# aaletov/open-pcc-metric

Hardware: AMD Instinct MI355X
Metric: Mpoints/s for symmetric D1+D2 PSNR, N_ref=N_deg=1M (higher is better)
Workload: dtype f64

## Files before the change

include/pccm.h:

```cpp
#ifndef PCCM_H
#define PCCM_H

#include <stdint.h>

#ifdef __cplusplus
extern "C" {
#endif

#define PCCM_VERSION 100

#define PCCM_OK 0
#define PCCM_E_ARG (-1)
#define PCCM_E_NODEV (-2)
#define PCCM_E_HIP (-3)
#define PCCM_E_OOM (-4)
#define PCCM_E_STATE (-5)
#define PCCM_E_RANGE (-6)

#define PCCM_F32 0
#define PCCM_F64 1

#define PCCM_DIR_LEFT 0
#define PCCM_DIR_RIGHT 1
#define PCCM_DIR_SELF 2
// ... 56 lines not shown
int pccm_nn_want_idx(pccm_ctx *ctx, int on);

int pccm_nn_fetch(pccm_ctx *ctx, int dir, int32_t *idx, double *d2);

int pccm_error_vectors(pccm_ctx *ctx, int dir, double *out);

int pccm_tie_exposure(pccm_ctx *ctx, int dir, int normal_mode, double out[8]);

int pccm_point_metric(pccm_ctx *ctx, int dir, int metric, int normal_mode, double *out);

int64_t pccm_xvec_len(int64_t n_iter);
int pccm_reduce_prefetch(pccm_ctx *ctx, int dir, int metric, int normal_mode);
int pccm_reduce_prefetch_many(pccm_ctx *ctx, int n, const int *dirs, const int *metrics, const int *normal_modes);
int pccm_reduce(pccm_ctx *ctx, int dir, int metric, int normal_mode, double *xvec, double *minmax);
int pccm_finish_sum(const double *xvec, int64_t n_iter, double *sum);
int pccm_reduce_total(pccm_ctx *ctx, int dir, int metric, int normal_mode, double out[3]);
int pccm_reduce_total_many(pccm_ctx *ctx, int n, const int *dirs, const int *metrics, const int *normal_modes, double *out);

int64_t pccm_cvec_len(int64_t n_iter);
int pccm_reduce_chunks_many(pccm_ctx *ctx, int n, const int *dirs, const int *metrics, const int *normal_modes, double *cvecs,
                            double *minmax);
int pccm_finish_chunks(const double *cvec, int64_t n_iter, double *sum);

int pccm_set_colors(pccm_ctx *ctx, int which, const void *rgb, int64_t n, int dtype, int on_device);

int pccm_set_colors_u8(pccm_ctx *ctx, int which, const unsigned char *rgb, int64_t n);

int pccm_color_reduce(pccm_ctx *ctx, int dir, int scheme, double scale, const int32_t *rows, int64_t nrows,
                      double sum_out[3], double max_out[3]);

int pccm_color_rows(pccm_ctx *ctx, int dir, int scheme, double scale, int what, const int32_t *rows, int64_t nrows,
                    double *out);

int pccm_obb_frames(pccm_ctx *ctx, const double *verts, int64_t nv, const double *tri, int64_t nt, double ext_out[3], double *vol_out);

int pccm_extreme_rows(pccm_ctx *ctx, int which, const float *dirs, int ndirs, int32_t *rows_out);
int pccm_rows_outside(pccm_ctx *ctx, int which, const double *planes, int nplanes, double margin, int32_t *rows_out, int64_t *count);

int pccm_seq_colsum(pccm_ctx *ctx, const double *cols, int64_t n, double out[3]);

int pccm_lzf_decompress(const unsigned char *in, int64_t in_len, unsigned char *out, int64_t out_cap, int64_t *out_len);

int pccm_color_transform(const double *rgb, int64_t n, int scheme, double *out);

int pccm_drop_caches(pccm_ctx *ctx);

// ... 19 lines not shown
```

open_pcc_metric_amd/_native.py:

```python
from __future__ import annotations

import ctypes
import os
import sys
import threading
from typing import Optional, Tuple

import numpy as np

_HERE = os.path.dirname(os.path.abspath(__file__))
LIB_PATH = os.environ.get("PCCM_LIB") or os.path.join(_HERE, "csrc", "libpccm.so")

OK, E_ARG, E_NODEV, E_HIP, E_OOM, E_STATE, E_RANGE = 0, -1, -2, -3, -4, -5, -6
F32, F64 = 0, 1
DIR_LEFT, DIR_RIGHT, DIR_SELF = 0, 1, 2
ENGINES = {"auto": 0, "brute": 1, "grid": 2}
NORMAL_MODES = {"row": 0, "neighbour": 1}
METRIC_D1, METRIC_D2, METRIC_PROJ = 0, 1, 2
KERNEL_CLASSES = {"ingest": 0, "scan": 1, "refine": 2, "fallback": 3, "point": 4, "reduce": 5,
                  "grid_build": 6, "grid_query": 7, "grid_finish": 8}

SYMBOLS = (
    "pccm_version", "pccm_last_error", "pccm_device_count", "pccm_ctx_create", "pccm_ctx_destroy", "pccm_ctx_reset",
    "pccm_set_cloud", "pccm_set_normals", "pccm_set_normals_deferred", "pccm_flush_uploads", "pccm_set_io_staged", "pccm_estimate_normals", "pccm_get_normals", "pccm_set_shard", "pccm_set_shard_dir", "pccm_shard_range", "pccm_nn", "pccm_nn_pair", "pccm_nn_fuse", "pccm_nn_want_idx", "pccm_nn_fetch",
    "pccm_error_vectors", "pccm_point_metric", "pccm_tie_exposure", "pccm_xvec_len", "pccm_reduce_prefetch", "pccm_reduce_prefetch_many", "pccm_reduce", "pccm_finish_sum",
    "pccm_reduce_total", "pccm_reduce_total_many", "pccm_cvec_len", "pccm_reduce_chunks_many", "pccm_finish_chunks",
    "pccm_set_colors", "pccm_set_colors_u8", "pccm_color_reduce", "pccm_color_rows", "pccm_seq_colsum", "pccm_obb_frames", "pccm_extreme_rows", "pccm_rows_outside",
    "pccm_color_transform", "pccm_lzf_decompress", "pccm_drop_caches", "pccm_graph_begin", "pccm_graph_end", "pccm_graph_launch", "pccm_graph_destroy",
    "pccm_sync",
    "pccm_profile_enable", "pccm_profile_reset", "pccm_profile_get", "pccm_nn_stats",
)

COLOR_SCHEMES = {"rgb": 0, "ycc": 1, "yuv": 2}
COLOR_OWN, COLOR_NEIGHBOUR, COLOR_DIFF, COLOR_SQUARE = 0, 1, 2, 3

_lib = None


class NativeLibraryMissing(ImportError):
    pass


class PccmStateError(RuntimeError):
    """PCCM_E_STATE: a call came in the wrong order or hit a stale object (a hipGraph captured before buffers
    changed, a reduction before its search).  The context is intact; callers may recover (CloudPair re-captures)."""


class PccmDeviceError(RuntimeError):
    """PCCM_E_HIP / PCCM_E_NODEV: the HIP runtime reported a failure.  Never retried, never swallowed."""
# ... 6 lines not shown
    if not os.path.exists(LIB_PATH):
        raise NativeLibraryMissing(
            f"{LIB_PATH} is not built: open_pcc_metric_amd has no CPU fallback. "
            "Run `make -C open_pcc_metric_amd/csrc` (needs hipcc, --offload-arch=gfx950).")
    if "torch" in sys.modules or os.environ.get("PCCM_NO_TORCH") != "1":
        try:
            import torch
        except ImportError:
            pass
    lib = ctypes.CDLL(LIB_PATH)
    vp, i32, i64 = ctypes.c_void_p, ctypes.c_int, ctypes.c_int64
    dp = ctypes.POINTER(ctypes.c_double)
    lib.pccm_version.restype = i32
    lib.pccm_last_error.restype = ctypes.c_char_p
    lib.pccm_device_count.argtypes = [ctypes.POINTER(i32)]
    lib.pccm_ctx_create.argtypes = [i32, vp, ctypes.POINTER(vp)]
    lib.pccm_ctx_destroy.argtypes = [vp]
    lib.pccm_ctx_reset.argtypes = [vp]
    lib.pccm_set_cloud.argtypes = [vp, i32, vp, i64, i32, i32]
    lib.pccm_set_normals.argtypes = [vp, i32, vp, i64, i32, i32]
    lib.pccm_set_normals_deferred.argtypes = [vp, i32, vp, i64, i32]
    lib.pccm_flush_uploads.argtypes = [vp]
    lib.pccm_set_io_staged.argtypes = [vp, i32]
    lib.pccm_set_shard.argtypes = [vp, i32, i32]
    lib.pccm_set_shard_dir.argtypes = [vp, i32, i32, i32]
    lib.pccm_estimate_normals.argtypes = [vp, i32, i32]
    lib.pccm_get_normals.argtypes = [vp, i32, vp]
    lib.pccm_shard_range.argtypes = [vp, i32, ctypes.POINTER(i64), ctypes.POINTER(i64)]
    lib.pccm_nn.argtypes = [vp, i32, i32]
    lib.pccm_nn_pair.argtypes = [vp, i32]
    lib.pccm_nn_fuse.argtypes = [vp, i32, i32]
    lib.pccm_nn_want_idx.argtypes = [vp, i32]
    lib.pccm_nn_fetch.argtypes = [vp, i32, vp, vp]
    lib.pccm_error_vectors.argtypes = [vp, i32, vp]
    lib.pccm_point_metric.argtypes = [vp, i32, i32, i32, vp]
    lib.pccm_tie_exposure.argtypes = [vp, i32, i32, dp]
    lib.pccm_xvec_len.argtypes = [i64]
    lib.pccm_xvec_len.restype = i64
    lib.pccm_reduce.argtypes = [vp, i32, i32, i32, vp, vp]
    lib.pccm_reduce_prefetch.argtypes = [vp, i32, i32, i32]
    ip = ctypes.POINTER(i32)
    lib.pccm_reduce_prefetch_many.argtypes = [vp, i32, ip, ip, ip]
    lib.pccm_finish_sum.argtypes = [vp, i64, dp]
    lib.pccm_reduce_total.argtypes = [vp, i32, i32, i32, dp]
    lib.pccm_reduce_total_many.argtypes = [vp, i32, ip, ip, ip, dp]
    lib.pccm_cvec_len.argtypes = [i64]
# ... 200 lines not shown
        self._n = [0, 0]

    def set_cloud(self, which: int, points) -> None:
        ptr, n, dt, dev, keep = _as_rows(points, "points")
        _check(self._lib.pccm_set_cloud(self._ctx, int(which), ptr, n, dt, dev))
        self._n[which] = n

    def set_normals(self, which: int, normals) -> None:
        ptr, n, dt, dev, keep = _as_rows(normals, "normals")
        self.__dict__.setdefault("_deferred", {}).pop(int(which), None)
        _check(self._lib.pccm_set_normals(self._ctx, int(which), ptr, n, dt, dev))

    def set_normals_deferred(self, which: int, normals) -> None:
        ptr, n, dt, dev, keep = _as_rows(normals, "normals")
        if dev:
            _check(self._lib.pccm_set_normals(self._ctx, int(which), ptr, n, dt, dev))
            return
        _check(self._lib.pccm_set_normals_deferred(self._ctx, int(which), ptr, n, dt))
        self.__dict__.setdefault("_deferred", {})[int(which)] = keep

    def set_io_staged(self, on: bool) -> None:
        _check(self._lib.pccm_set_io_staged(self._ctx, 1 if on else 0))

    def flush_uploads(self) -> None:
        try:
            _check(self._lib.pccm_flush_uploads(self._ctx))
        finally:
            self.__dict__.get("_deferred", {}).clear()

    def set_colors(self, which: int, colors) -> None:
        ptr, n, dt, dev, keep = _as_rows(colors, "colors")
        _check(self._lib.pccm_set_colors(self._ctx, int(which), ptr, n, dt, dev))

    def set_colors_u8(self, which: int, colors_u8) -> None:
        c = np.ascontiguousarray(colors_u8, dtype=np.uint8)
        if c.ndim != 2 or c.shape[1] != 3:
            raise ValueError("colors_u8 must have shape (N, 3)")
        _check(self._lib.pccm_set_colors_u8(self._ctx, int(which), c.ctypes.data_as(ctypes.c_void_p), c.shape[0]))

    @staticmethod
    def _rows_arg(rows):
        if rows is None:
            return None, 0, None
        keep = np.ascontiguousarray(rows, dtype=np.int32)
        return keep.ctypes.data_as(ctypes.c_void_p), keep.shape[0], keep

# ... 200 lines not shown
```

open_pcc_metric_amd/csrc/pccm_api.hip:

```cpp
#include <math.h>
#include <stdarg.h>
#include <stdio.h>
#include <string.h>

#include <new>
#include <thread>

#include "pccm_internal.h"

namespace pccm {

static thread_local char g_err[512] = "";

int fail(int code, const char *fmt, ...)
{
    va_list ap;
    va_start(ap, fmt);
    vsnprintf(g_err, sizeof(g_err), fmt, ap);
    va_end(ap);
    return code;
}

int ensure(pccm_ctx *ctx, DevBuf &b, size_t bytes)
{
    if (bytes <= b.bytes && b.p) return PCCM_OK;
    if (ctx->capturing) {
        ctx->capture_failed = true;
// ... 356 lines not shown
    if (!out) return fail(PCCM_E_ARG, "null pointer");
    *out = nullptr;
    int c = 0;
    if (hipGetDeviceCount(&c) != hipSuccess || c <= 0) {
        (void)hipGetLastError();
        return fail(PCCM_E_NODEV, "no HIP device is visible: libpccm has no CPU path");
    }
    if (device < 0 || device >= c) return fail(PCCM_E_ARG, "device %d out of range (0..%d)", device, c - 1);
    PCCM_HIP(hipSetDevice(device));
    pccm_ctx *ctx = new (std::nothrow) pccm_ctx();
    if (!ctx) return fail(PCCM_E_OOM, "host allocation failed");
    ctx->device = device;
    if (hip_stream) {
        ctx->stream = (hipStream_t)hip_stream;
    } else {
        hipError_t e = hipStreamCreateWithFlags(&ctx->stream, hipStreamNonBlocking);
        if (e != hipSuccess) {
            delete ctx;
            return fail(PCCM_E_HIP, "hipStreamCreate: %s", hipGetErrorString(e));
        }
        ctx->own_stream = true;
    }
    int rc = ensure(ctx, ctx->counters, 16 * sizeof(uint32_t));
    if (!rc && hipHostMalloc((void **)&ctx->host_err, 64, hipHostMallocDefault) != hipSuccess) {
        ctx->host_err = nullptr;
        rc = fail(PCCM_E_OOM, "hipHostMalloc of the device error word failed");
    }
    if (!rc) *ctx->host_err = 0u;
    if (!rc && hipEventCreateWithFlags(&ctx->batch_ev, hipEventDisableTiming) != hipSuccess) rc = fail(PCCM_E_HIP, "hipEventCreate failed");
    if (!rc) rc = ensure(ctx, ctx->stats, 32 * sizeof(unsigned long long));
    if (!rc && hipMemsetAsync(ctx->counters.p, 0, 16 * sizeof(uint32_t), ctx->stream) != hipSuccess)
        rc = fail(PCCM_E_HIP, "hipMemsetAsync failed");
    if (rc) {
        pccm_ctx_destroy(ctx);
        return rc;
    }
    for (int d = 0; d < 3; ++d) ctx->nn[d].nflag_dev = (uint32_t *)ctx->counters.p + 2 * d;
    *out = ctx;
    return PCCM_OK;
}

int pccm_ctx_destroy(pccm_ctx *ctx)
{
    if (!ctx) return PCCM_OK;
    (void)hipSetDevice(ctx->device);
    if (ctx->stream) (void)hipStreamSynchronize(ctx->stream);
    for (auto &s : ctx->spans) {
        (void)hipEventDestroy(s.a);
        (void)hipEventDestroy(s.b);
    }
    for (auto e : ctx->event_pool) (void)hipEventDestroy(e);
    if (ctx->batch_ev) (void)hipEventDestroy(ctx->batch_ev);
    ctx->batch_ev = nullptr;
    if (ctx->host_err) (void)hipHostFree(ctx->host_err);
    ctx->host_err = nullptr;
    for (int k = 0; k < 2; ++k) free_cloud(ctx->cloud[k]);
    for (int d = 0; d < 3; ++d) free_nn(ctx->nn[d]);
    DevBuf *bufs[] = {&ctx->part_b1, &ctx->part_g, &ctx->part_b2, &ctx->val, &ctx->stats, &ctx->staging, &ctx->staging2,
                      &ctx->counters, &ctx->color_cols, &ctx->color_idx, &ctx->colsum_scratch, &ctx->rescan_part, &ctx->tail_sync};
    for (DevBuf *b : bufs) free_buf(*b);
    for (auto &g : ctx->graphs) graph_free(g);
    for (auto &s : ctx->slots) {
        free_buf(s.val);
        if (s.host) (void)hipHostFree(s.host);
        if (s.ev) (void)hipEventDestroy(s.ev);
        s.ev = s.wait_ev = nullptr;
    }
    grid_release(ctx);
    if (ctx->copy_stream) (void)hipStreamDestroy(ctx->copy_stream);
    for (auto &pbuf : ctx->pin)
        if (pbuf) (void)hipHostFree(pbuf);
    for (auto &pe : ctx->pin_ev)
        if (pe) (void)hipEventDestroy(pe);
    if (ctx->own_stream && ctx->stream) (void)hipStreamDestroy(ctx->stream);
    delete ctx;
    return PCCM_OK;
}

// ... 85 lines not shown
    if (!nrm || n <= 0) return fail(PCCM_E_ARG, "empty normals");
    if (dtype != PCCM_F32 && dtype != PCCM_F64) return fail(PCCM_E_ARG, "dtype must be PCCM_F32 or PCCM_F64");
    Cloud &c = ctx->cloud[which];
    PCCM_HIP(hipStreamSynchronize(ctx->stream));
    for (int d = 0; d < 3; ++d) ctx->nn_gen[d]++;
    ctx->epoch++;
    c.nrm_exact32 = false;
    int rc = grow((void **)&c.nrm64, c.cap_nrm, (size_t)n * 3 * sizeof(double));
    if (rc) return rc;
    if ((rc = grow((void **)&c.nrm32, c.cap_nrm32, (size_t)n * sizeof(float4)))) return rc;
    c.n_nrm = n;
    c.nrm_host = nrm;
    c.nrm_host_dtype = dtype;
    c.nrm_deferred = true;
    return PCCM_OK;
}

int pccm_set_io_staged(pccm_ctx *ctx, int on)
{
    CHECK_CTX(ctx);
    NOT_CAPTURING(ctx);
    PCCM_HIP(hipStreamSynchronize(ctx->stream));
    ctx->io_staged = on != 0;
    return PCCM_OK;
}

int pccm_flush_uploads(pccm_ctx *ctx)
{
    CHECK_CTX(ctx);
    NOT_CAPTURING(ctx);
    for (int k = 0; k < 2; ++k) {
        int rc = normals_ready(ctx, ctx->cloud[k]);
        if (rc) return rc;
    }
    return PCCM_OK;
}

int pccm_set_colors(pccm_ctx *ctx, int which, const void *rgb, int64_t n, int dtype, int on_device)
{
    CHECK_CTX(ctx);
    NOT_CAPTURING(ctx);
    if (which != 0 && which != 1) return fail(PCCM_E_ARG, "cloud index must be 0 or 1");
    if (!rgb || n <= 0) return fail(PCCM_E_ARG, "empty colours");
    if (dtype != PCCM_F32 && dtype != PCCM_F64) return fail(PCCM_E_ARG, "dtype must be PCCM_F32 or PCCM_F64");
    Cloud &c = ctx->cloud[which];
    if (c.n == 0) return fail(PCCM_E_STATE, "set cloud %d before its colours", which);
// ... 584 lines not shown
    return tie_exposure(ctx, dir, *it, *se, *res, normal_mode, out);
}

int pccm_point_metric(pccm_ctx *ctx, int dir, int metric, int normal_mode, double *out)
{
    CHECK_CTX(ctx);
    NOT_CAPTURING(ctx);
    if (!out) return fail(PCCM_E_ARG, "null pointer");
    const double *dev;
    int64_t ns;
    const Cloud *it;
    NNResult *res;
    int rc = metric_on_device(ctx, dir, metric, normal_mode, &dev, &ns, &it, &res);
    if (rc) return rc;
    if (ns > 0) { int rcd = d2h(ctx, out, dev, (size_t)ns * sizeof(double)); if (rcd) return rcd; }
    PCCM_HIP(hipStreamSynchronize(ctx->stream));
    return PCCM_OK;
}

int64_t pccm_xvec_len(int64_t n_iter)
{
    if (n_iter <= 0) return 0;
    return (n_iter / kChunk) * (kChunk / kLeaf) + (n_iter % kChunk);
}

static int slot_prepare(pccm_ctx *ctx, ReduceSlot &s, int dir, int metric, int normal_mode, bool want_units, PointJobs &pj,
                        UnitJobs &uj)
{
    const Cloud *it, *se;
    NNResult *res;
    int rc = need_nn(ctx, dir, &it, &se, &res);
    if (rc) return rc;
    const int64_t ns = res->end - res->begin;
    const double *dev = nullptr;
    int stride = 1, square = 0, defer = 0;
    if (metric == PCCM_METRIC_D1) {
        if (res->rec_valid) {
            dev = (const double *)res->rec.p;
            stride = res->rec_stride;
            if (res->rec_layout == 1) defer = 3;
        } else {
            if ((rc = ensure_plain(ctx, *res, false))) return rc;
            dev = res->d2;
        }
    } else {
        if (metric != PCCM_METRIC_D2 && metric != PCCM_METRIC_PROJ) return fail(PCCM_E_ARG, "bad metric %d", metric);
// ... 17 lines not shown
                pj.off[pj.njobs + 1] = pj.off[pj.njobs] + ns;
                pj.njobs++;
            }
        }
    }
    s.dir = dir; s.metric = metric; s.mode = normal_mode;
    s.gen = ctx->nn_gen[dir];
    s.n_iter = it->n; s.begin = res->begin; s.end = res->end;
    s.nunits = ns > 0 ? (ns + kLeaf - 1) / kLeaf : 0;
    s.nblocks = (s.nunits + 31) / 32;
    s.has_units = want_units;
    const int64_t nfull = it->n / kChunk, full_rows = nfull * kChunk;
    s.t0 = res->begin > full_rows ? res->begin : full_rows;
    s.tail_n = s.t0 < res->end ? res->end - s.t0 : 0;
    const size_t need = (size_t)(3 * s.nunits + 3 * s.nblocks + s.tail_n + 1) * sizeof(double);
    if (ctx->capturing && (need > s.host_cap || !s.ev)) {
        ctx->capture_failed = true;
        return fail(PCCM_E_STATE, "a reduction slot must be allocated during graph capture: run the sequence once first");
    }
    if (need > s.host_cap) {
        ctx->epoch++;
        if (s.host) (void)hipHostFree(s.host);
        s.host = nullptr; s.host_cap = 0;
        PCCM_HIP(hipHostMalloc((void **)&s.host, need, hipHostMallocDefault));
        s.host_cap = need;
    }
    if (!s.ev) PCCM_HIP(hipEventCreateWithFlags(&s.ev, hipEventDisableTiming));
    if (s.nunits > 0) {
        UnitCol col;
        col.off = (stride >= 2 && metric != PCCM_METRIC_D1) ? 1 : 0;
        col.square = square;
        col.out_units = want_units ? s.host : nullptr;
        col.out_blocks = s.host + 3 * s.nunits;
        col.out_tail = s.host + 3 * s.nunits + 3 * s.nblocks;
        const double *base = stride >= 2 ? (const double *)res->rec.p : dev;
        UnitJob *host_job = nullptr;
        static const bool merge = [] {
            const char *e = PCCM_DIAG_ENV("PCCM_REDUCE_MERGE");
            return !(e && e[0] == '0');
        }();
        if (stride >= 2 && merge)
            for (int k = 0; k < uj.njobs; ++k)
                if (uj.j[k].stride >= 2 && uj.j[k].val == base && uj.j[k].ncols == 1 &&
                    (uj.j[k].defer == defer || uj.j[k].defer == 3 || defer == 3))
                    host_job = &uj.j[k];
        if (host_job) {
            host_job->c[1] = col;
// ... 57 lines not shown
static int prefetch_many(pccm_ctx *ctx, int n, const int *dirs, const int *metrics, const int *normal_modes, bool want_units)
{
    if (n < 0 || n > 8 || (n > 0 && (!dirs || !metrics || !normal_modes))) return fail(PCCM_E_ARG, "1..8 requests expected");
    PointJobs pj;
    UnitJobs uj;
    pj.njobs = 0; pj.off[0] = 0;
    uj.njobs = 0; uj.uoff[0] = 0; uj.toff[0] = 0;
    ReduceSlot *fresh[8];
    int nfresh = 0;
    for (int k = 0; k < n; ++k) {
        if (dirs[k] < 0 || dirs[k] > 2) return fail(PCCM_E_ARG, "bad direction %d", dirs[k]);
        if (metrics[k] == PCCM_METRIC_D1 || dirs[k] == PCCM_DIR_SELF) continue;
        NNResult &res = ctx->nn[dirs[k]];
        if (!res.valid || !res.rec_valid || ((res.fused_mode == normal_modes[k] || res.rec_stride == 4 || res.rec_layout == 1) && !res.no_rows)) continue;
        if (slot_find(ctx, dirs[k], metrics[k], normal_modes[k], want_units)) continue;
        int rc = ensure_plain(ctx, res, true);
        if (rc) return rc;
    }
    for (int k = 0; k < n; ++k) {
        if (dirs[k] < 0 || dirs[k] > 2) return fail(PCCM_E_ARG, "bad direction %d", dirs[k]);
        if (slot_find(ctx, dirs[k], metrics[k], normal_modes[k], want_units)) continue;
        ReduceSlot *s = slot_free(ctx, fresh, nfresh);
        if (!s) return fail(PCCM_E_STATE, "no free reduction slot: more than 8 live columns in one batch");
        if (s->pending && !ctx->capturing && s->wait_ev) PCCM_HIP(hipEventSynchronize(s->wait_ev));
        s->pending = false;
        int rc = slot_prepare(ctx, *s, dirs[k], metrics[k], normal_modes[k], want_units, pj, uj);
        if (rc) return rc;
        s->pending = true;
        fresh[nfresh++] = s;
    }
    if (nfresh == 0) return PCCM_OK;
    int rc;
    if ((rc = launch_point_jobs(ctx, pj))) return rc;
    if ((rc = launch_unit_jobs(ctx, uj))) return rc;
    for (int k = 0; k < nfresh; ++k) {
        ReduceSlot &s = *fresh[k];
        if (ctx->capturing) {
            GraphOp op;
            op.kind = 2;
            op.dir = s.dir;
            op.slot = (int)(&s - ctx->slots);
            op.snap = s;
            ctx->cap_ops.push_back(op);
        } else {
            s.wait_ev = ctx->batch_ev;
        }
    }
    if (!ctx->capturing) PCCM_HIP(hipEventRecord(ctx->batch_ev, ctx->stream));
    return PCCM_OK;
}

int pccm_reduce_prefetch(pccm_ctx *ctx, int dir, int metric, int normal_mode)
{
    return pccm_reduce_prefetch_many(ctx, 1, &dir, &metric, &normal_mode);
}

int pccm_reduce(pccm_ctx *ctx, int dir, int metric, int normal_mode, double *xvec, double *minmax)
{
    CHECK_CTX(ctx);
    NOT_CAPTURING(ctx);
    if (!xvec || !minmax) return fail(PCCM_E_ARG, "null pointer");
    if (dir < 0 || dir > 2) return fail(PCCM_E_ARG, "bad direction %d", dir);
    ReduceSlot *s = slot_find(ctx, dir, metric, normal_mode, true);
    if (!s) {
        int rc = prefetch_many(ctx, 1, &dir, &metric, &normal_mode, true);
        if (rc) return rc;
        s = slot_find(ctx, dir, metric, normal_mode, true);
        if (!s) return fail(PCCM_E_STATE, "reduction slot lost");
    }
    if (s->wait_ev) PCCM_HIP(hipEventSynchronize(s->wait_ev));
    { int rce = check_device_errors(ctx); if (rce) return rce; }
    s->pending = false;
    const int64_t n = s->n_iter;
    const int64_t xlen = pccm_xvec_len(n);
    memset(xvec, 0, (size_t)xlen * sizeof(double));
    minmax[0] = INFINITY;
    minmax[1] = -INFINITY;
    const int64_t nunits = s->nunits;
    const int64_t nfull = n / kChunk, full_rows = nfull * kChunk;
    const double *usum = s->host, *umin = usum + nunits, *umax = usum + 2 * nunits;
    for (int64_t u = 0; u < nunits; ++u) {
        const int64_t row = s->begin + u * kLeaf;
        if (row < full_rows) xvec[row / kLeaf] = usum[u];
        if (umin[u] < minmax[0]) minmax[0] = umin[u];
        if (umax[u] > minmax[1]) minmax[1] = umax[u];
    }
    if (s->tail_n > 0)
        memcpy(xvec + nfull * (kChunk / kLeaf) + (s->t0 - full_rows), s->host + 3 * nunits + 3 * s->nblocks,
               (size_t)s->tail_n * sizeof(double));
    return PCCM_OK;
}

static double leaf_tree(const double *l, int cnt)
// ... 12 lines not shown
    for (int64_t c = 0; c < nfull; ++c) {
        double cs = leaf_tree(xvec + c * lpc, lpc);
        s = first ? cs : s + cs;
        first = false;
    }
    if (tail) {
        double ts = np_pairwise_sum(xvec + nfull * lpc, tail);
        s = first ? ts : s + ts;
    }
    *sum = s;
    return PCCM_OK;
}

static int total_from_slot(pccm_ctx *ctx, int dir, int metric, int normal_mode, double out[3])
{
    if (dir < 0 || dir > 2) return fail(PCCM_E_ARG, "bad direction %d", dir);
    ReduceSlot *s = slot_find(ctx, dir, metric, normal_mode);
    if (!s) {
        int rc = pccm_reduce_prefetch(ctx, dir, metric, normal_mode);
        if (rc) return rc;
        s = slot_find(ctx, dir, metric, normal_mode);
        if (!s) return fail(PCCM_E_STATE, "reduction slot lost");
    }
    if (s->wait_ev) PCCM_HIP(hipEventSynchronize(s->wait_ev));
    { int rce = check_device_errors(ctx); if (rce) return rce; }
    s->pending = false;
    const int64_t n = s->n_iter, nunits = s->nunits, nblocks = s->nblocks;
    const int64_t nfull = n / kChunk;
    const double *bsum = s->host + 3 * nunits, *bmin = bsum + nblocks, *bmax = bsum + 2 * nblocks;
    double total = 0.0;
    bool first = true;
    for (int64_t c = 0; c < nfull; ++c) {
        const double cs = bsum[2 * c] + bsum[2 * c + 1];
        total = first ? cs : total + cs;
        first = false;
    }
    if (s->tail_n > 0) {
        const double ts = np_pairwise_sum(s->host + 3 * nunits + 3 * nblocks, s->tail_n);
        total = first ? ts : total + ts;
    }
    double mn = INFINITY, mx = -INFINITY;
    for (int64_t b = 0; b < nblocks; ++b) {
        mn = bmin[b] < mn ? bmin[b] : mn;
        mx = bmax[b] > mx ? bmax[b] : mx;
    }
    out[0] = total;
    out[1] = mn;
    out[2] = mx;
    return PCCM_OK;
}

int64_t pccm_cvec_len(int64_t n_iter)
{
    if (n_iter <= 0) return 0;
    return n_iter / kChunk + n_iter % kChunk;
}

static int chunks_from_slot(pccm_ctx *ctx, int dir, int metric, int normal_mode, double *cvec, double minmax[2])
{
    if (dir < 0 || dir > 2) return fail(PCCM_E_ARG, "bad direction %d", dir);
    ReduceSlot *s = slot_find(ctx, dir, metric, normal_mode);
    if (!s) {
        int rc = prefetch_many(ctx, 1, &dir, &metric, &normal_mode, false);
        if (rc) return rc;
        s = slot_find(ctx, dir, metric, normal_mode);
        if (!s) return fail(PCCM_E_STATE, "reduction slot lost");
    }
    if (s->wait_ev) PCCM_HIP(hipEventSynchronize(s->wait_ev));
    { int rce = check_device_errors(ctx); if (rce) return rce; }
    s->pending = false;
    const int64_t n = s->n_iter, nunits = s->nunits, nblocks = s->nblocks;
    const int64_t nfull = n / kChunk, full_rows = nfull * kChunk;
    memset(cvec, 0, (size_t)pccm_cvec_len(n) * sizeof(double));
    minmax[0] = INFINITY;
    minmax[1] = -INFINITY;
    if (s->end <= s->begin) return PCCM_OK;
    if (s->begin % kChunk != 0 || (s->end % kChunk != 0 && s->end != n))
        return fail(PCCM_E_STATE, "rows [%lld, %lld) do not start and end on 8192-row chunks: use pccm_reduce", (long long)s->begin,
                    (long long)s->end);
    const double *bsum = s->host + 3 * nunits, *bmin = bsum + nblocks, *bmax = bsum + 2 * nblocks;
    const int64_t c0 = s->begin / kChunk;
    const int64_t owned = ((s->end < full_rows ? s->end : full_rows) - s->begin) / kChunk;
    for (int64_t c = 0; c < owned; ++c) cvec[c0 + c] = bsum[2 * c] + bsum[2 * c + 1];
    if (s->tail_n > 0)
        memcpy(cvec + nfull + (s->t0 - full_rows), s->host + 3 * nunits + 3 * nblocks, (size_t)s->tail_n * sizeof(double));
    for (int64_t b = 0; b < nblocks; ++b) {
        minmax[0] = bmin[b] < minmax[0] ? bmin[b] : minmax[0];
        minmax[1] = bmax[b] > minmax[1] ? bmax[b] : minmax[1];
    }
    return PCCM_OK;
}
// ... 125 lines not shown
    if (g.graph) (void)hipGraphDestroy(g.graph);
    g.exec = nullptr;
    g.graph = nullptr;
    g.valid = false;
    g.ops.clear();
}

static int graph_replay(pccm_ctx *ctx, GraphRec &g)
{

    for (auto &op : g.ops) {
        if (op.kind == 1) {
            ctx->nn_gen[op.dir]++;
            ctx->nn[op.dir].valid = true;
            ctx->nn[op.dir].rec_valid = op.rec_valid;
            ctx->nn[op.dir].plain_valid = op.plain_valid;
            ctx->nn[op.dir].fused_mode = op.fused_mode;
            ctx->nn[op.dir].rec_stride = op.rec_stride;
            ctx->nn[op.dir].rec_layout = op.rec_layout;
            ctx->nn[op.dir].no_rows = op.no_rows;
            ctx->nn[op.dir].plain_d2_valid = op.plain_valid;
        } else if (op.kind == 2) {
            ReduceSlot &s = ctx->slots[op.slot];
            if (s.pending && s.gen == ctx->nn_gen[s.dir] && s.wait_ev) PCCM_HIP(hipEventSynchronize(s.wait_ev));
            s.dir = op.snap.dir; s.metric = op.snap.metric; s.mode = op.snap.mode;
            s.n_iter = op.snap.n_iter; s.begin = op.snap.begin; s.end = op.snap.end;
            s.nunits = op.snap.nunits; s.nblocks = op.snap.nblocks; s.has_units = op.snap.has_units;
            s.t0 = op.snap.t0; s.tail_n = op.snap.tail_n;
            s.gen = ctx->nn_gen[s.dir];
            s.pending = true;
            s.wait_ev = ctx->batch_ev;
        }
    }
    PCCM_HIP(hipGraphLaunch(g.exec, ctx->stream));
    PCCM_HIP(hipEventRecord(ctx->batch_ev, ctx->stream));
    return PCCM_OK;
}

int pccm_graph_begin(pccm_ctx *ctx)
{
    CHECK_CTX(ctx);
    if (ctx->capturing) return fail(PCCM_E_STATE, "already capturing");
    PCCM_HIP(hipStreamSynchronize(ctx->stream));
    for (auto &s : ctx->slots) s.pending = false;
    ctx->cap_ops.clear();
    ctx->capture_failed = false;
    PCCM_HIP(hipStreamBeginCapture(ctx->stream, hipStreamCaptureModeThreadLocal));
    ctx->capturing = true;
    return PCCM_OK;
}

int pccm_graph_end(pccm_ctx *ctx, int *graph_id)
{
    CHECK_CTX(ctx);
    if (!graph_id) return fail(PCCM_E_ARG, "null pointer");
    if (!ctx->capturing) return fail(PCCM_E_STATE, "pccm_graph_begin was not called");
    ctx->capturing = false;
    GraphRec g;
    hipError_t e = hipStreamEndCapture(ctx->stream, &g.graph);
    if (e != hipSuccess || ctx->capture_failed || !g.graph) {
        (void)hipGetLastError();
        if (g.graph) (void)hipGraphDestroy(g.graph);
        for (int d = 0; d < 3; ++d) { ctx->nn[d].valid = false; ctx->nn_gen[d]++; }
        for (auto &s : ctx->slots) s.pending = false;
        grid_invalidate(ctx);
        return fail(PCCM_E_STATE, "graph capture failed (%s); the context is usable, results were invalidated",
                    e != hipSuccess ? hipGetErrorString(e) : "a captured call reported an error");
    }
    e = hipGraphInstantiate(&g.exec, g.graph, nullptr, nullptr, 0);
    if (e != hipSuccess) {
        (void)hipGraphDestroy(g.graph);
        for (int d = 0; d < 3; ++d) { ctx->nn[d].valid = false; ctx->nn_gen[d]++; }
        for (auto &s : ctx->slots) s.pending = false;
        grid_invalidate(ctx);
        return fail(PCCM_E_HIP, "hipGraphInstantiate: %s", hipGetErrorString(e));
    }
    g.ops = ctx->cap_ops;
    for (auto &op : g.ops)
        if (op.kind == 1) {
            op.rec_valid = ctx->nn[op.dir].rec_valid;
            op.plain_valid = ctx->nn[op.dir].plain_valid;
            op.fused_mode = ctx->nn[op.dir].fused_mode;
            op.rec_stride = ctx->nn[op.dir].rec_stride;
            op.rec_layout = ctx->nn[op.dir].rec_layout;
            op.no_rows = ctx->nn[op.dir].no_rows;
        }
    g.epoch = ctx->epoch;
    g.valid = true;
    PCCM_HIP(hipGraphLaunch(g.exec, ctx->stream));
    for (auto &op : g.ops)
        if (op.kind == 2) ctx->slots[op.slot].wait_ev = ctx->batch_ev;
    PCCM_HIP(hipEventRecord(ctx->batch_ev, ctx->stream));
    int id = -1;
    for (size_t k = 0; k < ctx->graphs.size(); ++k)
        if (!ctx->graphs[k].valid && !ctx->graphs[k].exec) { id = (int)k; break; }
    if (id < 0) { ctx->graphs.emplace_back(); id = (int)ctx->graphs.size() - 1; }
    ctx->graphs[id] = g;
    *graph_id = id;
    return PCCM_OK;
}

int pccm_graph_launch(pccm_ctx *ctx, int graph_id)
{
    CHECK_CTX(ctx);
    NOT_CAPTURING(ctx);
    if (graph_id < 0 || graph_id >= (int)ctx->graphs.size() || !ctx->graphs[graph_id].valid)
        return fail(PCCM_E_ARG, "unknown graph %d", graph_id);
    GraphRec &g = ctx->graphs[graph_id];
    if (g.epoch != ctx->epoch) {
        graph_free(g);
        return fail(PCCM_E_STATE, "graph %d is stale: inputs, shard or buffers changed since it was captured", graph_id);
    }
    return graph_replay(ctx, g);
}
// ... 111 lines not shown
```

open_pcc_metric_amd/csrc/pccm_internal.h:

```cpp
#pragma once
#include <hip/hip_runtime.h>
#include <stdint.h>
#include <mutex>
#include <string>
#include <vector>

#include "pccm.h"

#ifdef PCCM_DIAG
#define PCCM_DIAG_ENV(name) getenv(name)
#else
#define PCCM_DIAG_ENV(name) (static_cast<const char *>(nullptr))
#endif

namespace pccm {

constexpr int kScanThreads = 256;
constexpr int kScanTile = 1024;
constexpr int kTileVec = kScanTile / 4 * 3;
constexpr int kGranule = 64;
constexpr float kBig32 = 3.0e38f;
constexpr float kPadCoord = 1.0e18f;
constexpr double kMaxAbsCoord = 1.0e15;

// ... 105 lines not shown
    bool lattice = false;
    DevBuf occ;
    DevBuf recs;
    bool vox = false;
    DevBuf vbricks;
    DevBuf vlist;
    DevBuf vcount;
    bool vox_rows = false;
    uint64_t vox_rows_pair = 0;
    DevBuf vminrow;
};

struct ReduceSlot {
    bool pending = false;
    int dir = 0, metric = 0, mode = 0;
    uint64_t gen = 0;
    int64_t n_iter = 0, begin = 0, end = 0, nunits = 0, nblocks = 0, t0 = 0, tail_n = 0;
    bool has_units = false;
    DevBuf val;
    double *host = nullptr;
    size_t host_cap = 0;
    hipEvent_t ev = nullptr;
    hipEvent_t wait_ev = nullptr;
};

struct ProfSpan {
    hipEvent_t a, b;
    int cls;
};

struct GraphOp {
    int kind = 0;
    int dir = 0, slot = -1;
    bool rec_valid = false, plain_valid = false;
    int fused_mode = -1, rec_stride = 4, rec_layout = 0;
    bool no_rows = false;
    ReduceSlot snap;
};

struct GraphRec {
    hipGraph_t graph = nullptr;
    hipGraphExec_t exec = nullptr;
    std::vector<GraphOp> ops;
    uint64_t epoch = 0;
    bool valid = false;
};

}

struct pccm_ctx {
    std::recursive_mutex mu;
    int device = 0;
    hipStream_t stream = nullptr;
    bool own_stream = false;
    hipStream_t copy_stream = nullptr;
    pccm::DevBuf staging2;
    void *pin[3] = {nullptr, nullptr, nullptr};
    size_t pin_cap[3] = {0, 0, 0};
    hipEvent_t pin_ev[2] = {nullptr, nullptr};
    bool pin_ev_set[2] = {false, false};
    bool io_staged = false;
    pccm::Cloud cloud[2];
    int shard_rank[3] = {0, 0, 0}, shard_world[3] = {1, 1, 1};
    bool sharded() const { return shard_world[0] != 1 || shard_world[1] != 1 || shard_world[2] != 1; }
    pccm::NNResult nn[3];
    pccm::DevBuf part_b1, part_g, part_b2, val, stats, staging, counters;
    pccm::DevBuf rescan_part;
    pccm::DevBuf tail_sync;
    bool tail_sync_clean = false;
    pccm::DevBuf color_cols, color_idx;
    pccm::DevBuf colsum_scratch;
    bool colsum_configured = false;
    struct ColorMemo {
        bool valid = false, range_bad = false;
        int dir = 0, scheme = 0;
        double scale = 0.0, sum[3] = {0, 0, 0}, max[3] = {0, 0, 0};
        uint64_t gen = 0, rgb_gen = 0;
    } color_memo;
    uint64_t rgb_gen = 1;
    pccm::Grid grid;
    pccm::DevBuf g_cell_of, g_rank, g_hist, g_blocksum, g_qrecs;
    pccm::DevBuf g_bins, g_tmp;
    hipEvent_t batch_ev = nullptr;
    uint32_t *host_err = nullptr;
    bool bins_clean = false;
    int want_idx = 1;
    int fuse_mode[3] = {-1, -1, -1};
    pccm::ReduceSlot slots[8];
    uint64_t nn_gen[3] = {1, 1, 1};
    uint64_t epoch = 1;
    bool capturing = false, capture_failed = false;
    std::vector<pccm::GraphOp> cap_ops;
    std::vector<pccm::GraphRec> graphs;
    bool prof_on = false;
    std::vector<pccm::ProfSpan> spans;
    std::vector<hipEvent_t> event_pool;
    double prof_ms[PCCM_K_COUNT] = {0};
    int64_t prof_n[PCCM_K_COUNT] = {0};
};

namespace pccm {

int fail(int code, const char *fmt, ...);
#define PCCM_HIP(expr)                                                                        \
    do {                                                                                      \
        hipError_t _e = (expr);                                                               \
// ... 81 lines not shown
    int stride;
    int defer;
    int64_t nrm_rows;
    const double *nrm64;
    const float4 *nrm32;
    const float4 *q32;
    int64_t row0;
    int ncols;
    UnitCol c[2];
    int64_t ns, nunits;
    int64_t tail_first, tail_n;
    int64_t nblocks;
};
struct UnitJobs {
    UnitJob j[8];
    int njobs;
    int64_t uoff[9];
    int64_t toff[9];
};
int rescan_jobs(pccm_ctx *ctx, int njobs, const Cloud *const *its, const Cloud *const *ses, NNResult *const *ress, bool self, RescanJobs *out);
constexpr unsigned kRescanCap = 512;
int launch_point_jobs(pccm_ctx *ctx, const PointJobs &jobs);
int launch_unpack(pccm_ctx *ctx, const double *rec, int stride, int layout, const float4 *q32, int64_t row0, int64_t ns, int32_t *idx, double *d2);
int launch_unit_jobs(pccm_ctx *ctx, const UnitJobs &jobs);

int launch_point_metric(pccm_ctx *ctx, const Cloud &it, const Cloud &se, const NNResult &res, int metric,
                        int normal_mode, double *out_val , double *out_err );

double np_pairwise_sum(const double *a, int64_t n);

int launch_obb_frames(pccm_ctx *ctx, const double *verts, int64_t nv, const double *tri, int64_t nt, double *ext_out, double *vol_out);
int launch_extreme_rows(pccm_ctx *ctx, const double *x64, int64_t n, const float *dirs, int ndirs, unsigned long long *best);
int launch_outside_planes(pccm_ctx *ctx, const double *x64, int64_t n, const double *planes, int nplanes, double margin,
                          int32_t *rows_out, unsigned int *count);

int launch_rgb8(pccm_ctx *ctx, Cloud &c, const unsigned char *bytes, unsigned int *flag);
int launch_color_rows(pccm_ctx *ctx, const double *own, const double *other, const int32_t *rows, int64_t n,
                      int64_t n_other, int scheme, double scale, int what, double *out,
                      unsigned long long *maxkeys, unsigned int *bad, const uint32_t *own8 = nullptr, const uint32_t *other8 = nullptr,
                      const float4 *recs = nullptr);
int launch_color_colsum(pccm_ctx *ctx, const double *cols, int64_t n, double *out3);
int launch_color_colsums(pccm_ctx *ctx, int njobs, const double *const cols[2], const int64_t n[2], double *const out3[2],
                         unsigned long long *const outmax[2]);
int launch_colors_from_u8(pccm_ctx *ctx, const unsigned char *src, int64_t n3, double *out);

}
```

open_pcc_metric_amd/csrc/pccm_point.hip:

```cpp
#include "pccm_internal.h"

namespace pccm {

__device__ __forceinline__ unsigned long long order_key(double v)
{
    unsigned long long b = (unsigned long long)__double_as_longlong(v);
    return (b >> 63) ? ~b : (b | 0x8000000000000000ull);
}

template <typename T>
__global__ __launch_bounds__(256) void k_ingest_points(const T *__restrict__ src, int64_t n, int64_t n_pad,
                                                       float *__restrict__ x32, double *__restrict__ x64, float4 *__restrict__ x32r,
                                                       unsigned long long *__restrict__ stats)
{
    __shared__ unsigned long long s_mx[4], s_lo[4][3], s_hi[4][3];
    __shared__ int s_cnt[4][3];
    unsigned long long mx = 0;
    unsigned long long lo[3] = {~0ull, ~0ull, ~0ull}, hi[3] = {0ull, 0ull, 0ull};
    int inexact = 0, bad = 0, frac = 0;
    for (int64_t i = (int64_t)blockIdx.x * 256 + threadIdx.x; i < n_pad; i += (int64_t)gridDim.x * 256) {
        if (i < n) {
            double v[3];
            float f[3];
#pragma unroll
// ... 514 lines not shown
    const int64_t e = c0 - jobs.toff[jb];
    const double *p = J.val + (J.tail_first + e) * STRIDE;
    double w[NC];
    if (DEFER) {
        double x, y;
        matched_fields(*reinterpret_cast<const float4 *>(p), J.q32, DEFER, J.nrm64, J.nrm32, J.row0 + J.tail_first + e, CFG != 1, x, y, J.nrm_rows);
        if (CFG == 0) { w[0] = x; w[1] = __dmul_rn(y, y); }
        else if (CFG == 1) w[0] = x;
        else if (CFG == 2) w[0] = __dmul_rn(y, y);
        else w[0] = y;
    } else if (STRIDE >= 2) {
        const double2 q = *reinterpret_cast<const double2 *>(p);
        if (CFG == 0) { w[0] = q.x; w[1] = __dmul_rn(q.y, q.y); }
        else if (CFG == 1) w[0] = q.x;
        else if (CFG == 2) w[0] = __dmul_rn(q.y, q.y);
        else w[0] = q.y;
    } else {
        w[0] = *p;
    }
#pragma unroll
    for (int c = 0; c < NC; ++c) J.c[c].out_tail[e] = w[c];
}

static int job_shape(const UnitJob &J)
{
    int cfg = -1;
    if (J.stride == 1) cfg = (J.ncols == 1 && J.c[0].off == 0 && !J.c[0].square) ? 1 : -1;
    else if (J.ncols == 2) cfg = (J.c[0].off == 0 && !J.c[0].square && J.c[1].off == 1 && J.c[1].square) ? 0 : -1;
    else if (J.c[0].off == 0) cfg = J.c[0].square ? -1 : 1;
    else cfg = J.c[0].square ? 2 : 3;
    if (cfg < 0 || (J.stride != 1 && J.stride != 2 && J.stride != 4)) return -1;
    if (J.defer && J.stride != 2) return -1;
    return J.stride * 4 + cfg + 64 * J.defer;
}

static void launch_unit_shape(pccm_ctx *ctx, const UnitJobs &jobs, int shape)
{
    const int64_t total = jobs.uoff[jobs.njobs] + jobs.toff[jobs.njobs];
    const dim3 grid((unsigned)((total + 255) / 256)), block(256);
    switch (shape) {
    case 1 * 4 + 1: hipLaunchKernelGGL((k_unit_lean<1, 1>), grid, block, 0, ctx->stream, jobs); break;
    case 2 * 4 + 0: hipLaunchKernelGGL((k_unit_lean<2, 0>), grid, block, 0, ctx->stream, jobs); break;
    case 2 * 4 + 1: hipLaunchKernelGGL((k_unit_lean<2, 1>), grid, block, 0, ctx->stream, jobs); break;
    case 2 * 4 + 2: hipLaunchKernelGGL((k_unit_lean<2, 2>), grid, block, 0, ctx->stream, jobs); break;
    case 4 * 4 + 0: hipLaunchKernelGGL((k_unit_lean<4, 0>), grid, block, 0, ctx->stream, jobs); break;
    case 4 * 4 + 1: hipLaunchKernelGGL((k_unit_lean<4, 1>), grid, block, 0, ctx->stream, jobs); break;
// ... 2 lines not shown
    case 64 + 2 * 4 + 1: hipLaunchKernelGGL((k_unit_lean<2, 1, 1>), grid, block, 0, ctx->stream, jobs); break;
    case 64 + 2 * 4 + 2: hipLaunchKernelGGL((k_unit_lean<2, 2, 1>), grid, block, 0, ctx->stream, jobs); break;
    case 128 + 2 * 4 + 0: hipLaunchKernelGGL((k_unit_lean<2, 0, 2>), grid, block, 0, ctx->stream, jobs); break;
    case 128 + 2 * 4 + 1: hipLaunchKernelGGL((k_unit_lean<2, 1, 2>), grid, block, 0, ctx->stream, jobs); break;
    case 128 + 2 * 4 + 2: hipLaunchKernelGGL((k_unit_lean<2, 2, 2>), grid, block, 0, ctx->stream, jobs); break;
    case 192 + 2 * 4 + 1: hipLaunchKernelGGL((k_unit_lean<2, 1, 3>), grid, block, 0, ctx->stream, jobs); break;
    case 256 + 2 * 4 + 0: hipLaunchKernelGGL((k_unit_lean<2, 0, 4>), grid, block, 0, ctx->stream, jobs); break;
    case 256 + 2 * 4 + 2: hipLaunchKernelGGL((k_unit_lean<2, 2, 4>), grid, block, 0, ctx->stream, jobs); break;
    case 320 + 2 * 4 + 0: hipLaunchKernelGGL((k_unit_lean<2, 0, 5>), grid, block, 0, ctx->stream, jobs); break;
    case 320 + 2 * 4 + 2: hipLaunchKernelGGL((k_unit_lean<2, 2, 5>), grid, block, 0, ctx->stream, jobs); break;
    default: hipLaunchKernelGGL(k_unit_jobs, grid, block, 0, ctx->stream, jobs); break;
    }
}

static bool lean_has(int shape)
{
    switch (shape) {
    case 5: case 8: case 9: case 10: case 16: case 17: case 18: case 72: case 73: case 74: case 136: case 137: case 138: case 201: case 264: case 266:
    case 328: case 330: return true;
    default: return false;
    }
}

int launch_unit_jobs(pccm_ctx *ctx, const UnitJobs &jobs)
{
    const int64_t total = jobs.uoff[jobs.njobs] + jobs.toff[jobs.njobs];
    if (total <= 0) return PCCM_OK;
    ProfScope ps(ctx, PCCM_K_REDUCE);
    static const bool general = [] { const char *e = getenv("PCCM_REDUCE_GENERAL"); return e && e[0] == '1'; }();
    int shape[8], nshapes = 0, first_of[8];
    bool all_lean = !general;
    for (int k = 0; k < jobs.njobs; ++k) {
        shape[k] = job_shape(jobs.j[k]);
        all_lean = all_lean && lean_has(shape[k]);
        bool seen = false;
        for (int j = 0; j < nshapes; ++j) seen = seen || shape[first_of[j]] == shape[k];
        if (!seen) first_of[nshapes++] = k;
    }
    if (!all_lean) {
        launch_unit_shape(ctx, jobs, -1);
    } else if (nshapes == 1) {
        launch_unit_shape(ctx, jobs, shape[0]);
    } else {
        for (int g = 0; g < nshapes; ++g) {
            UnitJobs sub;
            sub.njobs = 0;
            sub.uoff[0] = sub.toff[0] = 0;
            for (int k = 0; k < jobs.njobs; ++k) {
                if (shape[k] != shape[first_of[g]]) continue;
                sub.j[sub.njobs] = jobs.j[k];
                sub.uoff[sub.njobs + 1] = sub.uoff[sub.njobs] + (jobs.uoff[k + 1] - jobs.uoff[k]);
                sub.toff[sub.njobs + 1] = sub.toff[sub.njobs] + (jobs.toff[k + 1] - jobs.toff[k]);
                sub.njobs++;
            }
            for (int k = sub.njobs; k < 8; ++k) {
                sub.j[k] = sub.j[0];
                sub.uoff[k + 1] = sub.uoff[sub.njobs];
                sub.toff[k + 1] = sub.toff[sub.njobs];
            }
            launch_unit_shape(ctx, sub, shape[first_of[g]]);
        }
    }
    PCCM_HIP(hipGetLastError());
    return PCCM_OK;
}

__global__ __launch_bounds__(256) void k_unpack(const double *__restrict__ rec, int stride, int layout, const float4 *__restrict__ q32, int64_t row0,
                                                int64_t ns, int32_t *__restrict__ idx, double *__restrict__ d2)
{
    const int64_t i = (int64_t)blockIdx.x * 256 + threadIdx.x;
    if (i >= ns) return;
    if (layout == 1) {
        const float4 r = reinterpret_cast<const float4 *>(rec)[i];
        double x, y;
        matched_fields(r, q32, 3, nullptr, nullptr, row0 + i, false, x, y);
        if (idx) idx[i] = __float_as_int(r.w);
        d2[i] = x;
        return;
    }
    const double *r = rec + i * stride;
    if (stride == 4 && idx) idx[i] = (int32_t)(__double_as_longlong(r[2]) & 0xffffffffll);
    d2[i] = r[0];
}

int launch_unpack(pccm_ctx *ctx, const double *rec, int stride, int layout, const float4 *q32, int64_t row0, int64_t ns, int32_t *idx, double *d2)
// ... 31 lines not shown
```

Measured before the change: 10290.

## Spin on device-published completion counter instead of blocking event sync

Adds a tiny kernel after each reduction batch that atomically increments a host-coherent counter, and replaces hipEventSynchronize on reduction slots with a bounded host spin on that counter, falling back to the event. It also switches the slot host buffers to coherent host memory. The aim is to cut the wake-up latency of blocking event waits for small reductions. In exchange it adds one kernel launch per batch, burns a CPU core while waiting, and uncached coherent memory may slow host reads of results.

```diff
diff --git a/include/pccm.h b/include/pccm.h
--- a/include/pccm.h
+++ b/include/pccm.h
@@ -102,6 +102,11 @@
                             double *minmax);
 int pccm_finish_chunks(const double *cvec, int64_t n_iter, double *sum);
 
+#define PCCM_WAIT_SPIN 0
+#define PCCM_WAIT_EVENT 1
+int pccm_set_wait(pccm_ctx *ctx, int mode);
+int pccm_wait_counter(pccm_ctx *ctx, uint64_t *out);
+
 int pccm_set_colors(pccm_ctx *ctx, int which, const void *rgb, int64_t n, int dtype, int on_device);
 
 int pccm_set_colors_u8(pccm_ctx *ctx, int which, const unsigned char *rgb, int64_t n);
diff --git a/open_pcc_metric_amd/_native.py b/open_pcc_metric_amd/_native.py
--- a/open_pcc_metric_amd/_native.py
+++ b/open_pcc_metric_amd/_native.py
@@ -25,6 +25,7 @@
     "pccm_set_cloud", "pccm_set_normals", "pccm_set_normals_deferred", "pccm_flush_uploads", "pccm_set_io_staged", "pccm_estimate_normals", "pccm_get_normals", "pccm_set_shard", "pccm_set_shard_dir", "pccm_shard_range", "pccm_nn", "pccm_nn_pair", "pccm_nn_fuse", "pccm_nn_want_idx", "pccm_nn_fetch",
     "pccm_error_vectors", "pccm_point_metric", "pccm_tie_exposure", "pccm_xvec_len", "pccm_reduce_prefetch", "pccm_reduce_prefetch_many", "pccm_reduce", "pccm_finish_sum",
     "pccm_reduce_total", "pccm_reduce_total_many", "pccm_cvec_len", "pccm_reduce_chunks_many", "pccm_finish_chunks",
+    "pccm_set_wait", "pccm_wait_counter",
     "pccm_set_colors", "pccm_set_colors_u8", "pccm_color_reduce", "pccm_color_rows", "pccm_seq_colsum", "pccm_obb_frames", "pccm_extreme_rows", "pccm_rows_outside",
     "pccm_color_transform", "pccm_lzf_decompress", "pccm_drop_caches", "pccm_graph_begin", "pccm_graph_end", "pccm_graph_launch", "pccm_graph_destroy",
     "pccm_sync",
@@ -77,6 +78,8 @@
     lib.pccm_set_normals_deferred.argtypes = [vp, i32, vp, i64, i32]
     lib.pccm_flush_uploads.argtypes = [vp]
     lib.pccm_set_io_staged.argtypes = [vp, i32]
+    lib.pccm_set_wait.argtypes = [vp, i32]
+    lib.pccm_wait_counter.argtypes = [vp, ctypes.POINTER(ctypes.c_uint64)]
     lib.pccm_set_shard.argtypes = [vp, i32, i32]
     lib.pccm_set_shard_dir.argtypes = [vp, i32, i32, i32]
     lib.pccm_estimate_normals.argtypes = [vp, i32, i32]
@@ -323,6 +326,17 @@
     def set_io_staged(self, on: bool) -> None:
         _check(self._lib.pccm_set_io_staged(self._ctx, 1 if on else 0))
 
+    def set_wait(self, mode: str) -> None:
+        modes = {"spin": 0, "event": 1}
+        if mode not in modes:
+            raise ValueError(f"wait mode {mode!r}: expected one of {sorted(modes)}")
+        _check(self._lib.pccm_set_wait(self._ctx, modes[mode]))
+
+    def wait_counter(self) -> int:
+        out = ctypes.c_uint64(0)
+        _check(self._lib.pccm_wait_counter(self._ctx, ctypes.byref(out)))
+        return int(out.value)
+
     def flush_uploads(self) -> None:
         try:
             _check(self._lib.pccm_flush_uploads(self._ctx))
diff --git a/open_pcc_metric_amd/csrc/pccm_api.hip b/open_pcc_metric_amd/csrc/pccm_api.hip
--- a/open_pcc_metric_amd/csrc/pccm_api.hip
+++ b/open_pcc_metric_amd/csrc/pccm_api.hip
@@ -3,6 +3,7 @@
 #include <stdio.h>
 #include <string.h>
 
+#include <chrono>
 #include <new>
 #include <thread>
 
@@ -405,11 +406,16 @@
         ctx->own_stream = true;
     }
     int rc = ensure(ctx, ctx->counters, 16 * sizeof(uint32_t));
-    if (!rc && hipHostMalloc((void **)&ctx->host_err, 64, hipHostMallocDefault) != hipSuccess) {
+    if (!rc && hipHostMalloc((void **)&ctx->host_err, 64, hipHostMallocCoherent) != hipSuccess) {
         ctx->host_err = nullptr;
         rc = fail(PCCM_E_OOM, "hipHostMalloc of the device error word failed");
     }
     if (!rc) *ctx->host_err = 0u;
+    if (!rc && hipHostMalloc((void **)&ctx->done, 128, hipHostMallocCoherent) != hipSuccess) {
+        ctx->done = nullptr;
+        rc = fail(PCCM_E_OOM, "hipHostMalloc of the completion counter failed");
+    }
+    if (!rc) *ctx->done = 0;
     if (!rc && hipEventCreateWithFlags(&ctx->batch_ev, hipEventDisableTiming) != hipSuccess) rc = fail(PCCM_E_HIP, "hipEventCreate failed");
     if (!rc) rc = ensure(ctx, ctx->stats, 32 * sizeof(unsigned long long));
     if (!rc && hipMemsetAsync(ctx->counters.p, 0, 16 * sizeof(uint32_t), ctx->stream) != hipSuccess)
@@ -437,6 +443,8 @@
     ctx->batch_ev = nullptr;
     if (ctx->host_err) (void)hipHostFree(ctx->host_err);
     ctx->host_err = nullptr;
+    if (ctx->done) (void)hipHostFree(ctx->done);
+    ctx->done = nullptr;
     for (int k = 0; k < 2; ++k) free_cloud(ctx->cloud[k]);
     for (int d = 0; d < 3; ++d) free_nn(ctx->nn[d]);
     DevBuf *bufs[] = {&ctx->part_b1, &ctx->part_g, &ctx->part_b2, &ctx->val, &ctx->stats, &ctx->staging, &ctx->staging2,
@@ -568,6 +576,25 @@
     NOT_CAPTURING(ctx);
     PCCM_HIP(hipStreamSynchronize(ctx->stream));
     ctx->io_staged = on != 0;
+    return PCCM_OK;
+}
+
+int pccm_set_wait(pccm_ctx *ctx, int mode)
+{
+    CHECK_CTX(ctx);
+#ifdef PCCM_DIAG
+    if (mode == 2) { ctx->wait_mode = mode; return PCCM_OK; }
+#endif
+    if (mode != PCCM_WAIT_SPIN && mode != PCCM_WAIT_EVENT) return fail(PCCM_E_ARG, "bad wait mode %d", mode);
+    ctx->wait_mode = mode;
+    return PCCM_OK;
+}
+
+int pccm_wait_counter(pccm_ctx *ctx, uint64_t *out)
+{
+    CHECK_CTX(ctx);
+    if (!out) return fail(PCCM_E_ARG, "null pointer");
+    *out = __atomic_load_n(ctx->done, __ATOMIC_ACQUIRE);
     return PCCM_OK;
 }
 
@@ -1198,6 +1225,31 @@
 {
     if (n_iter <= 0) return 0;
     return (n_iter / kChunk) * (kChunk / kLeaf) + (n_iter % kChunk);
+}
+
+
+static int wait_slot(pccm_ctx *ctx, const ReduceSlot *s)
+{
+    constexpr auto kSpinBound = std::chrono::milliseconds(2);
+    const uint64_t want = s->wait_seq;
+    if (ctx->wait_mode == PCCM_WAIT_SPIN && want) {
+        const auto t0 = std::chrono::steady_clock::now();
+        for (unsigned k = 0;; ++k) {
+            if (__atomic_load_n(ctx->done, __ATOMIC_ACQUIRE) >= want) return PCCM_OK;
+            __builtin_ia32_pause();
+            if ((k & 255) == 255 && std::chrono::steady_clock::now() - t0 > kSpinBound) break;
+        }
+    }
+#ifdef PCCM_DIAG
+    if (ctx->wait_mode == 2 && s->wait_ev) {
+        hipError_t e;
+        while ((e = hipEventQuery(s->wait_ev)) == hipErrorNotReady) __builtin_ia32_pause();
+        PCCM_HIP(e);
+        return PCCM_OK;
+    }
+#endif
+    if (s->wait_ev) PCCM_HIP(hipEventSynchronize(s->wait_ev));
+    return PCCM_OK;
 }
 
 static int slot_prepare(pccm_ctx *ctx, ReduceSlot &s, int dir, int metric, int normal_mode, bool want_units, PointJobs &pj,
@@ -1261,7 +1313,7 @@
         ctx->epoch++;
         if (s.host) (void)hipHostFree(s.host);
         s.host = nullptr; s.host_cap = 0;
-        PCCM_HIP(hipHostMalloc((void **)&s.host, need, hipHostMallocDefault));
+        PCCM_HIP(hipHostMalloc((void **)&s.host, need, hipHostMallocCoherent));
         s.host_cap = need;
     }
     if (!s.ev) PCCM_HIP(hipEventCreateWithFlags(&s.ev, hipEventDisableTiming));
@@ -1365,7 +1417,7 @@
         if (slot_find(ctx, dirs[k], metrics[k], normal_modes[k], want_units)) continue;
         ReduceSlot *s = slot_free(ctx, fresh, nfresh);
         if (!s) return fail(PCCM_E_STATE, "no free reduction slot: more than 8 live columns in one batch");
-        if (s->pending && !ctx->capturing && s->wait_ev) PCCM_HIP(hipEventSynchronize(s->wait_ev));
+        if (s->pending && !ctx->capturing && s->wait_ev) { int rcw = wait_slot(ctx, s); if (rcw) return rcw; }
         s->pending = false;
         int rc = slot_prepare(ctx, *s, dirs[k], metrics[k], normal_modes[k], want_units, pj, uj);
         if (rc) return rc;
@@ -1375,9 +1427,11 @@
     if (nfresh == 0) return PCCM_OK;
     int rc;
     if ((rc = launch_point_jobs(ctx, pj))) return rc;
-    if ((rc = launch_unit_jobs(ctx, uj))) return rc;
+    uint64_t seq = 0;
+    if ((rc = launch_unit_jobs(ctx, uj, &seq))) return rc;
     for (int k = 0; k < nfresh; ++k) {
         ReduceSlot &s = *fresh[k];
+        s.wait_seq = seq;
         if (ctx->capturing) {
             GraphOp op;
             op.kind = 2;
@@ -1411,7 +1465,7 @@
         s = slot_find(ctx, dir, metric, normal_mode, true);
         if (!s) return fail(PCCM_E_STATE, "reduction slot lost");
     }
-    if (s->wait_ev) PCCM_HIP(hipEventSynchronize(s->wait_ev));
+    { int rcw = wait_slot(ctx, s); if (rcw) return rcw; }
     { int rce = check_device_errors(ctx); if (rce) return rce; }
     s->pending = false;
     const int64_t n = s->n_iter;
@@ -1470,7 +1524,7 @@
         s = slot_find(ctx, dir, metric, normal_mode);
         if (!s) return fail(PCCM_E_STATE, "reduction slot lost");
     }
-    if (s->wait_ev) PCCM_HIP(hipEventSynchronize(s->wait_ev));
+    { int rcw = wait_slot(ctx, s); if (rcw) return rcw; }
     { int rce = check_device_errors(ctx); if (rce) return rce; }
     s->pending = false;
     const int64_t n = s->n_iter, nunits = s->nunits, nblocks = s->nblocks;
@@ -1514,7 +1568,7 @@
         s = slot_find(ctx, dir, metric, normal_mode);
         if (!s) return fail(PCCM_E_STATE, "reduction slot lost");
     }
-    if (s->wait_ev) PCCM_HIP(hipEventSynchronize(s->wait_ev));
+    { int rcw = wait_slot(ctx, s); if (rcw) return rcw; }
     { int rce = check_device_errors(ctx); if (rce) return rce; }
     s->pending = false;
     const int64_t n = s->n_iter, nunits = s->nunits, nblocks = s->nblocks;
@@ -1686,7 +1740,10 @@
             ctx->nn[op.dir].plain_d2_valid = op.plain_valid;
         } else if (op.kind == 2) {
             ReduceSlot &s = ctx->slots[op.slot];
-            if (s.pending && s.gen == ctx->nn_gen[s.dir] && s.wait_ev) PCCM_HIP(hipEventSynchronize(s.wait_ev));
+            if (s.pending && s.gen == ctx->nn_gen[s.dir] && s.wait_ev) {
+                int rcw = wait_slot(ctx, &s);
+                if (rcw) return rcw;
+            }
             s.dir = op.snap.dir; s.metric = op.snap.metric; s.mode = op.snap.mode;
             s.n_iter = op.snap.n_iter; s.begin = op.snap.begin; s.end = op.snap.end;
             s.nunits = op.snap.nunits; s.nblocks = op.snap.nblocks; s.has_units = op.snap.has_units;
@@ -1694,8 +1751,10 @@
             s.gen = ctx->nn_gen[s.dir];
             s.pending = true;
             s.wait_ev = ctx->batch_ev;
+            s.wait_seq = op.snap.wait_seq ? ctx->batches_issued + op.snap.wait_seq : 0;
         }
     }
+    ctx->batches_issued += g.batches;
     PCCM_HIP(hipGraphLaunch(g.exec, ctx->stream));
     PCCM_HIP(hipEventRecord(ctx->batch_ev, ctx->stream));
     return PCCM_OK;
@@ -1708,6 +1767,7 @@
     PCCM_HIP(hipStreamSynchronize(ctx->stream));
     for (auto &s : ctx->slots) s.pending = false;
     ctx->cap_ops.clear();
+    ctx->cap_batches = 0;
     ctx->capture_failed = false;
     PCCM_HIP(hipStreamBeginCapture(ctx->stream, hipStreamCaptureModeThreadLocal));
     ctx->capturing = true;
@@ -1750,10 +1810,15 @@
             op.no_rows = ctx->nn[op.dir].no_rows;
         }
     g.epoch = ctx->epoch;
+    g.batches = ctx->cap_batches;
     g.valid = true;
+    for (auto &op : g.ops)
+        if (op.kind == 2) {
+            ctx->slots[op.slot].wait_ev = ctx->batch_ev;
+            ctx->slots[op.slot].wait_seq = op.snap.wait_seq ? ctx->batches_issued + op.snap.wait_seq : 0;
+        }
+    ctx->batches_issued += g.batches;
     PCCM_HIP(hipGraphLaunch(g.exec, ctx->stream));
-    for (auto &op : g.ops)
-        if (op.kind == 2) ctx->slots[op.slot].wait_ev = ctx->batch_ev;
     PCCM_HIP(hipEventRecord(ctx->batch_ev, ctx->stream));
     int id = -1;
     for (size_t k = 0; k < ctx->graphs.size(); ++k)
diff --git a/open_pcc_metric_amd/csrc/pccm_internal.h b/open_pcc_metric_amd/csrc/pccm_internal.h
--- a/open_pcc_metric_amd/csrc/pccm_internal.h
+++ b/open_pcc_metric_amd/csrc/pccm_internal.h
@@ -151,6 +151,7 @@
     size_t host_cap = 0;
     hipEvent_t ev = nullptr;
     hipEvent_t wait_ev = nullptr;
+    uint64_t wait_seq = 0;
 };
 
 struct ProfSpan {
@@ -172,6 +173,7 @@
     hipGraphExec_t exec = nullptr;
     std::vector<GraphOp> ops;
     uint64_t epoch = 0;
+    uint64_t batches = 0;
     bool valid = false;
 };
 
@@ -211,6 +213,10 @@
     pccm::DevBuf g_cell_of, g_rank, g_hist, g_blocksum, g_qrecs;
     pccm::DevBuf g_bins, g_tmp;
     hipEvent_t batch_ev = nullptr;
+    uint64_t *done = nullptr;
+    uint64_t batches_issued = 0;
+    uint64_t cap_batches = 0;
+    int wait_mode = PCCM_WAIT_SPIN;
     uint32_t *host_err = nullptr;
     bool bins_clean = false;
     int want_idx = 1;
@@ -338,7 +344,7 @@
 constexpr unsigned kRescanCap = 512;
 int launch_point_jobs(pccm_ctx *ctx, const PointJobs &jobs);
 int launch_unpack(pccm_ctx *ctx, const double *rec, int stride, int layout, const float4 *q32, int64_t row0, int64_t ns, int32_t *idx, double *d2);
-int launch_unit_jobs(pccm_ctx *ctx, const UnitJobs &jobs);
+int launch_unit_jobs(pccm_ctx *ctx, const UnitJobs &jobs, uint64_t *seq);
 
 int launch_point_metric(pccm_ctx *ctx, const Cloud &it, const Cloud &se, const NNResult &res, int metric,
                         int normal_mode, double *out_val , double *out_err );
diff --git a/open_pcc_metric_amd/csrc/pccm_point.hip b/open_pcc_metric_amd/csrc/pccm_point.hip
--- a/open_pcc_metric_amd/csrc/pccm_point.hip
+++ b/open_pcc_metric_amd/csrc/pccm_point.hip
@@ -560,6 +560,15 @@
     for (int c = 0; c < NC; ++c) J.c[c].out_tail[e] = w[c];
 }
 
+__global__ __launch_bounds__(64) void k_publish(unsigned long long *done)
+{
+    if (threadIdx.x == 0) {
+        __builtin_amdgcn_fence(__ATOMIC_RELEASE, "");
+        asm volatile("s_waitcnt vmcnt(0)" ::: "memory");
+        __hip_atomic_fetch_add(done, 1ull, __ATOMIC_RELAXED, __HIP_MEMORY_SCOPE_SYSTEM);
+    }
+}
+
 static int job_shape(const UnitJob &J)
 {
     int cfg = -1;
@@ -608,8 +617,9 @@
     }
 }
 
-int launch_unit_jobs(pccm_ctx *ctx, const UnitJobs &jobs)
-{
+int launch_unit_jobs(pccm_ctx *ctx, const UnitJobs &jobs, uint64_t *seq)
+{
+    *seq = 0;
     const int64_t total = jobs.uoff[jobs.njobs] + jobs.toff[jobs.njobs];
     if (total <= 0) return PCCM_OK;
     ProfScope ps(ctx, PCCM_K_REDUCE);
@@ -647,6 +657,8 @@
             launch_unit_shape(ctx, sub, shape[first_of[g]]);
         }
     }
+    *seq = ctx->capturing ? ++ctx->cap_batches : ++ctx->batches_issued;
+    hipLaunchKernelGGL(k_publish, dim3(1), dim3(64), 0, ctx->stream, (unsigned long long *)ctx->done);
     PCCM_HIP(hipGetLastError());
     return PCCM_OK;
 }
```

Measured after the change: 10940 (median of 6 runs). 6.4% higher.
